# mic-rud/Learned-Compression-of-Point-Cloud-Geometry-and-Attributes

Hardware: AMD Instinct MI355X
Metric: encode+decode Mpoints/sec (higher is better)
Workload: dtype f32

## Files before the change

### include/pcc_hip.h

```cpp
#ifndef PCC_HIP_H
#define PCC_HIP_H

#include <stdint.h>

#ifdef __cplusplus
extern "C" {
#endif

#define PCC_OK 0
#define PCC_ERR_ARG (-1)
#define PCC_ERR_HIP (-2)
#define PCC_ERR_UNSUPPORTED (-3)
#define PCC_ERR_DATA (-4)

#define PCC_ACT_NONE 0
#define PCC_ACT_RELU 1
#define PCC_ACT_LEAKY_RELU 2

int pcc_version(void);
const char* pcc_last_error(void);
int pcc_device_count(void);
int pcc_device_name(int dev, char* out, int out_len);

int64_t pcc_hash_capacity(int64_t n);

#define PCC_COORD_LIMIT 130000
#define PCC_BATCH_LIMIT 1022
#define PCC_COUNT_ERR_RANGE (-2)

int pcc_hash_build(const int32_t* coords, int64_t n, uint64_t* keys, int32_t* vals, int64_t cap,
                   int32_t tensor_stride, int32_t* dup_count, void* stream);

int pcc_hash_lookup(const uint64_t* keys, const int32_t* vals, int64_t cap, int32_t tensor_stride,
                    const int32_t* query, int64_t nq, int32_t* out_idx, void* stream);

int64_t pcc_scan_scratch_elems(int64_t m);

int pcc_stride_map(const int32_t* coords, int64_t n, int32_t ts, uint64_t* keys, int32_t* vals,
                   int64_t cap, int32_t* scratch, int32_t* out_coords, int64_t* out_count,
                   void* stream);

int pcc_children(const int32_t* coords, int64_t n, int32_t ts, int32_t ksize, uint64_t* keys,
                 int32_t* vals, int64_t cap, int32_t* scratch, int32_t* out_coords,
                 int64_t* out_count, void* stream);

int pcc_augment_rotate(const int32_t* coords, int64_t n, const float* rot, int32_t nbatch, float half,
                       uint64_t* keys, int32_t* vals, int64_t cap, int32_t* scratch, int32_t* out_coords,
                       int32_t* out_src, int64_t* out_count, void* stream);

int32_t pcc_color_jitter_chunk(void);
int64_t pcc_color_jitter_scratch_bytes(int64_t n, int32_t nbatch);
int pcc_color_jitter(const float* rgb, int64_t n, const int64_t* offsets, int32_t nbatch, const float* params,
                     const int32_t* order, float* out, void* scratch, int64_t scratch_bytes, void* stream);

int pcc_voxelize(const float* xyz, const int32_t* batch, int64_t n, int32_t nbatch, const float* attr, int32_t c,
                 float origin_x, float origin_y, float origin_z, float voxel, int32_t rounding, uint64_t* keys,
                 int32_t* vals, int64_t cap, int32_t* scratch, int32_t* out_coords, int32_t* out_first,
                 int32_t* out_npts, int64_t* out_sum, int32_t* out_row, int64_t* out_count, void* stream);

int pcc_kernel_map(const int32_t* out_coords, int64_t n_out, const uint64_t* in_keys,
                   const int32_t* in_vals, int64_t in_cap, int32_t ksize, int32_t step,
                   int32_t sign, int32_t* nbr, uint32_t* row_mask, int64_t* pair_count,
                   void* stream);

int pcc_pair_count(const uint32_t* row_mask, int64_t n_out, int64_t* pair_count, void* stream);

int64_t pcc_order_scratch_bytes(int64_t n);
int pcc_order_rows_by_mask(const uint32_t* row_mask, const int32_t* coords, int64_t n,
                           int32_t block_log2, int32_t tensor_stride, int32_t* order, uint32_t* group_mask32,
                           void* scratch, int64_t scratch_bytes, void* stream);
int pcc_permute_map_rows(const int32_t* nbr, const int32_t* order, int64_t n, int32_t K, int32_t* nbr_sorted, void* stream);

int64_t pcc_small_map_max(void);
int32_t pcc_small_paths(int32_t mask);
int pcc_small_kernel_map(const int32_t* out_coords, int64_t n_out, const uint64_t* in_keys, const int32_t* in_vals, int64_t in_cap,
                         int32_t ksize, int32_t step, int32_t sign, int32_t* nbr, uint32_t* row_mask, int32_t* order,
                         uint32_t* group_mask32, void* scratch, int64_t scratch_bytes, void* stream);

int64_t pcc_conv_packed_elems(int32_t K, int32_t cin, int32_t cout);
int pcc_conv_pack_weights(const float* w, int32_t K, int32_t cin, int32_t cout, float* w_packed,
                          void* stream);
int pcc_conv_fwd(const float* fin, int64_t n_in, int32_t cin, const float* w, const float* w_packed,
                 const float* bias, const int32_t* nbr, const int32_t* order,
                 const uint32_t* group_mask32, int32_t K, float* fout, int64_t n_out, int32_t cout,
                 int32_t act, const float* film, const float* residual, void* stream);

int64_t pcc_conv_small_max(int64_t workgroups);

int pcc_conv_kernel_name(int32_t mode, int64_t n_in, int32_t cin, int32_t cout, int64_t n_out, int32_t K, int32_t has_nbr,
                         char* buf, int32_t len);

int64_t pcc_conv_packed_elems_bf16(int32_t K, int32_t cin, int32_t cout);
int pcc_conv_pack_weights_bf16(const float* w, int32_t K, int32_t cin, int32_t cout, uint16_t* w_packed, void* stream);
int pcc_conv_fwd_bf16(const uint16_t* fin, int64_t n_in, int32_t cin, const uint16_t* w_packed, const float* bias,
                      const int32_t* nbr, const int32_t* order, const uint32_t* group_mask32, int32_t K, float* fout,
                      int64_t n_out, int32_t cout, int32_t act, const float* film, const float* residual, void* stream);

int pcc_epilogue_fwd(const float* c, const float* film, const float* residual, int64_t n, int32_t channels, int32_t act,
                     float* out, void* stream);
int pcc_epilogue_bwd(const float* dout, const float* c, const float* film, int64_t n, int32_t channels, int32_t act,
                     float* dc, float* dfilm, void* stream);

int64_t pcc_cast_colsum_scratch_elems(int32_t channels);
int pcc_cast_colsum(const float* x, int64_t n, int32_t channels, uint16_t* out_bf16, float* colsum, float* scratch,
                    int64_t scratch_elems, void* stream);

int64_t pcc_conv_packed_elems_x3(int32_t K, int32_t cin, int32_t cout);
int pcc_conv_pack_weights_x3(const float* w, int32_t K, int32_t cin, int32_t cout, uint16_t* w_packed, void* stream);
int pcc_conv_fwd_x3(const float* fin, int64_t n_in, int32_t cin, const uint16_t* w_packed, const float* bias,
                    const int32_t* nbr, const int32_t* order, const uint32_t* group_mask32, int32_t K, float* fout,
                    int64_t n_out, int32_t cout, int32_t act, const float* film, const float* residual, void* stream);

int pcc_im2col_thin(const float* fin, int32_t cin, const int32_t* nbr, int64_t n_out, int32_t K, float* out, int32_t k2,
                    void* stream);

int pcc_gather_sum_fwd(const float* scores, int32_t ld, const int32_t* nbr, int32_t K, int32_t cout,
                       const float* bias, float* out, int64_t n_out, int32_t act, void* stream);

int pcc_gather_rows(const float* src, int32_t c, const int32_t* idx, int64_t n, float* out,
                    int32_t accumulate, void* stream);

int pcc_scatter_rows(const float* src, int32_t c, const int32_t* idx, int64_t n, float* out,
                     void* stream);
int pcc_scatter_add_rows(const float* src, int32_t c, const int32_t* idx, int64_t n, float* out,
                         void* stream);

int pcc_compact_rows(const uint8_t* mask, int64_t n, const int32_t* coords, int32_t* out_coords,
                     const float* feats, int32_t c, float* out_feats, int32_t* new_index,
                     int32_t* scratch, int64_t* out_count, void* stream);

int64_t pcc_topk_state_elems(int32_t nbatch);
int pcc_topk_mask(const float* logits, int32_t ld, const int32_t* coords, int64_t n, int32_t nbatch,
                  const int32_t* k, uint8_t* mask, int32_t* state, void* stream);

int pcc_count_per_batch(const int32_t* coords, int64_t n, int32_t nbatch, int32_t* counts, void* stream);

int64_t pcc_sort_scratch_bytes(int64_t n);
int pcc_sort_coords(const int32_t* coords, int64_t n, int32_t* perm, void* scratch,
                    int64_t scratch_bytes, void* stream);

int pcc_kernel_map_transpose(const int32_t* nbr, int64_t n_out, int32_t K, int64_t n_in, int32_t* nbr_t,
                             uint32_t* row_mask_t, void* stream);
int64_t pcc_conv_wgrad_scratch_elems(int32_t K, int32_t cin, int32_t cout);
int pcc_conv_wgrad(const float* fin, int64_t n_in, int32_t cin, const float* dy, int64_t n_out, int32_t cout,
                   const int32_t* nbr, const int32_t* order, const uint32_t* group_mask32, int32_t K, float* dw,
                   float* scratch, int64_t scratch_elems, void* stream);
int pcc_conv_wgrad_kernel_name(int32_t bf16, int32_t K, int32_t cin, int32_t cout, int64_t n_out, char* buf, int32_t len,
                               int32_t* split, int32_t* partials);
int pcc_conv_wgrad_bf16(const uint16_t* fin, int64_t n_in, int32_t cin, const uint16_t* dy, int64_t n_out, int32_t cout,
                        const int32_t* nbr, const int32_t* order, const uint32_t* group_mask32, int32_t K, float* dw,
                        float* scratch, int64_t scratch_elems, void* stream);

int pcc_chconv(const float* x, int64_t n, int32_t c, const int32_t* coords, const uint64_t* keys, const int32_t* vals,
               int64_t cap, int32_t tensor_stride, int32_t ksize, const float* w, int32_t w_channels, int32_t flip,
               float* y, void* stream);

int64_t pcc_octree_scratch_bytes(int64_t n);
int pcc_octree_occupancy(const int32_t* coords, int64_t n, int32_t stride, const int32_t* origin,
                         int32_t depth, uint8_t* occupancy, int32_t* level_counts, void* scratch,
                         int64_t scratch_bytes, void* stream);
int pcc_octree_expand(const uint8_t* occupancy, const int64_t* level_counts, int32_t depth,
                      int32_t stride, const int32_t* origin, int32_t batch, int64_t n_points,
                      int32_t* coords_out, void* scratch, int64_t scratch_bytes, void* stream);

int pcc_nn_search(const int32_t* query, int64_t nq, const uint64_t* keys, const int32_t* vals, int64_t cap,
                  int32_t tensor_stride, const double* target_rgb, int32_t max_radius, int32_t* nn_idx, int64_t* nn_d2,
                  int32_t* tie_count, double* tie_rgb, void* stream);

int pcc_estimate_normals(const int32_t* coords, int64_t n, const uint64_t* keys, const int32_t* vals, int64_t cap,
                         int32_t tensor_stride, int32_t radius, int32_t orient_mode, const double* orient,
                         double* normals, int32_t* count, int64_t* moments, void* stream);

int64_t pcc_render_scratch_bytes(int32_t H, int32_t W);
int pcc_render_view(const int32_t* coords, const uint8_t* rgb8, int64_t n, const int32_t* right, const int32_t* up,
                    const int32_t* front, int32_t u_min, int32_t v_max, int32_t ox, int32_t oy, int32_t scale,
                    int32_t point_size, int32_t H, int32_t W, const uint8_t* background, void* scratch,
                    int64_t scratch_bytes, uint8_t* image, void* stream);
int32_t pcc_image_compare_tile(void);
int64_t pcc_image_compare_scratch_bytes(int32_t H, int32_t W);
int pcc_image_compare(const uint8_t* ref, const uint8_t* img, int32_t H, int32_t W, void* scratch,
                      int64_t scratch_bytes, double* out, void* stream);

int pcc_eb_quantize(const float* z, int64_t n, int32_t c, const float* medians, int32_t* symbols,
                    float* z_hat, void* stream);
int pcc_eb_dequantize(const int32_t* symbols, int64_t n, int32_t c, const float* medians,
                      float* z_hat, void* stream);
int pcc_eb_likelihood(const float* z_hat, int64_t n, int32_t c, const float* eb_params, float* lik,
                      void* stream);
int pcc_gc_encode_prep(const float* y, const float* params, int64_t n, int32_t c,
                       const float* scale_table, int32_t levels, int32_t* symbols,
                       int32_t* indexes, void* stream);
int pcc_gc_encode_prep_packed(const float* y, const float* params, int64_t n, int32_t c,
                              const float* scale_table, int32_t levels, const int32_t* perm,
                              int16_t* symbols, uint8_t* indexes, int32_t* overflow, void* stream);
int pcc_gc_dequantize_i16(const int16_t* symbols, const float* params, int64_t n, int32_t c,
                          float* y_hat, void* stream);
int pcc_gc_dequantize(const int32_t* symbols, const float* params, int64_t n, int32_t c, float* y_hat,
                      void* stream);
int pcc_gc_forward(const float* y, const float* params, int64_t n, int32_t c, float* y_hat, float* lik,
                   void* stream);

int64_t pcc_rans_encode_with_indexes(const int32_t* symbols, const int32_t* indexes, int64_t n,
                                     const int32_t* cdfs, int32_t cdf_stride, const int32_t* cdf_sizes,
                                     const int32_t* offsets, uint8_t* out, int64_t out_cap);
int pcc_rans_decode_with_indexes(const uint8_t* data, int64_t nbytes, const int32_t* indexes, int64_t n,
                                 const int32_t* cdfs, int32_t cdf_stride, const int32_t* cdf_sizes,
                                 const int32_t* offsets, int32_t* out_symbols);
int64_t pcc_rans_encode_with_indexes_i16u8(const int16_t* symbols, const uint8_t* indexes, int64_t n,
                                           const int32_t* cdfs, int32_t cdf_stride, const int32_t* cdf_sizes,
                                           const int32_t* offsets, uint8_t* out, int64_t out_cap);
int pcc_rans_decode_with_indexes_u8i16(const uint8_t* data, int64_t nbytes, const uint8_t* indexes, int64_t n,
                                       const int32_t* cdfs, int32_t cdf_stride, const int32_t* cdf_sizes,
                                       const int32_t* offsets, int16_t* out_symbols, int32_t* narrowed);
int pcc_pmf_to_quantized_cdf(const float* pmf, int32_t n, int32_t precision, int32_t* cdf);

int64_t pcc_rans_lanes_header(const uint8_t* data, int64_t nbytes);
int64_t pcc_rans_lanes_encode_host(const int32_t* symbols, const int32_t* indexes, int64_t n, int32_t lanes,
                                   const int32_t* cdfs, int32_t cdf_stride, const int32_t* cdf_sizes,
                                   const int32_t* offsets, uint8_t* out, int64_t out_cap);
int pcc_rans_lanes_decode_host(const uint8_t* data, int64_t nbytes, const int32_t* indexes, int64_t n,
                               const int32_t* cdfs, int32_t cdf_stride, const int32_t* cdf_sizes,
                               const int32_t* offsets, int32_t* out_symbols);
int64_t pcc_rans_lanes_tables_bytes(const int32_t* cdf_sizes, int32_t n_tables);
int pcc_rans_lanes_tables_build(const int32_t* cdfs, int32_t cdf_stride, const int32_t* cdf_sizes,
                                const int32_t* offsets, int32_t n_tables, void* out, int64_t out_bytes);
int64_t pcc_rans_lanes_encode_scratch_bytes(int64_t n, int32_t lanes, int32_t worst_case);
int64_t pcc_rans_lanes_encode_out_bytes(int64_t n, int32_t lanes, int32_t worst_case);
int pcc_rans_lanes_encode(const int32_t* symbols, const int32_t* indexes, int64_t n, int32_t lanes,
                          const void* tables, int32_t worst_case, void* scratch, int64_t scratch_bytes,
                          uint8_t* out, int64_t out_cap, int32_t* result, void* stream);
// ... 8 lines not shown
```

### learned-compression-of-point-cloud-geometry-and-attributes_amd/_build.py

```python
import os
import subprocess

_HERE = os.path.dirname(os.path.abspath(__file__))
SO_PATH = os.path.join(_HERE, "libpcc_hip.so")

NO_SCRATCH = {
    "conv": ("conv_small_kernel", "conv_mfma_buf_kernel", "conv_mfma_kernel"),
    "rans_lanes": ("rans_lanes_encode_kernel", "rans_lanes_pack_kernel", "rans_lanes_decode_kernel"),
    "chconv": ("chconv_kernel",),
    "augment": ("jitter_partial_kernel", "jitter_mean_kernel", "jitter_apply_kernel", "first_rows_clear_kernel",
                "first_rows_insert_kernel", "first_rows_flag_kernel", "first_rows_finalize_kernel"),
    "normals": ("estimate_normals_kernel",),
    "voxelize": ("first_rows_clear_kernel", "first_rows_insert_kernel", "first_rows_flag_kernel", "first_rows_finalize_kernel",
                 "voxelize_accumulate_kernel"),
}


def build(force=False):
    args = ["make", "-s", "-C", os.path.join(_HERE, "csrc"), "-j4"]
    if force:
        subprocess.check_call(args + ["clean"])
    subprocess.check_call(args)
    for stem, kernels in NO_SCRATCH.items():
        check_kernel_resources(os.path.join(_HERE, "build", stem + ".resources.txt"), kernels)
    check_small_kernel_lds_reads()
    return SO_PATH


def check_small_kernel_lds_reads(obj=None):
    import glob
    import shutil
    objdump = "/opt/rocm/lib/llvm/bin/llvm-objdump"
    obj = obj or os.path.join(_HERE, "build", "conv.o")
    if not os.path.exists(objdump) or not os.path.exists(obj):
        raise RuntimeError(f"cannot lint conv_small_kernel: {objdump} or {obj} is missing")
    tmp = os.path.join(_HERE, "build", "_lint")
    shutil.rmtree(tmp, ignore_errors=True)
    os.makedirs(tmp)
    local = os.path.join(tmp, "conv.o")
    shutil.copy(obj, local)
    subprocess.run([objdump, "--offloading", local], check=True, capture_output=True, cwd=tmp)
    cos = [f for f in glob.glob(local + ".*") if "amdgcn" in f]
    if not cos:
        raise RuntimeError("cannot lint conv_small_kernel: no device code object in build/conv.o")
    dis = subprocess.run([objdump, "-d", cos[0]], check=True, capture_output=True, text=True).stdout
    shutil.rmtree(tmp, ignore_errors=True)
    return lint_lds_reads(dis)


def lint_lds_reads(dis, kernel="conv_small_kernel"):
    import re

    def regs(operand):
        m = re.fullmatch(r"v\[(\d+):(\d+)\]", operand)
        if m:
            return set(range(int(m.group(1)), int(m.group(2)) + 1))
        m = re.fullmatch(r"v(\d+)", operand)
        return {int(m.group(1))} if m else set()

    checked, func, pending = 0, None, {}
    for line in dis.splitlines():
        m = re.match(r"^[0-9a-f]+ <(\S+)>:", line)
        if m:
            func = m.group(1) if kernel in m.group(1) else None
            pending = {}
            continue
        if func is None:
            continue
        text = line.split("//")[0].strip()
        if not text:
            continue
        parts = text.split(None, 1)
        mnem = parts[0]
        ops = [o.strip().split(" ")[0] for o in parts[1].split(",")] if len(parts) > 1 else []
        if mnem == "s_waitcnt" and "lgkmcnt(0)" in text:
            pending = {}
            continue
        touched = set()
        for o in ops:
            touched |= regs(o)
        clash = touched & set(pending)
        if mnem == "ds_read_b128":
            dest = regs(ops[0])
            clash = (touched - dest) & set(pending) | (dest & set(pending))
            if not clash:
                for r_ in dest:
                    pending[r_] = text
                checked += 1
        if clash:
            raise RuntimeError(f"{func}: `{text}` touches v{sorted(clash)} while an LDS read into them is still in flight "
                               f"(`{pending[sorted(clash)[0]]}`): the hand-placed s_waitcnt of conv_small_kernel no longer covers it")
    if not checked:
        raise RuntimeError(f"cannot lint {kernel}: no ds_read_b128 found in its disassembly")
    return checked


def check_kernel_resources(path=None, kernels=None):
    import re
    kernels = kernels or NO_SCRATCH["conv"]
    path = path or os.path.join(_HERE, "build", "conv.resources.txt")
    if not os.path.exists(path):
        raise RuntimeError(f"{path} is missing: the library was not built by csrc/Makefile")
    seen, name = {}, None
    vals = {}
    with open(path) as f:
        for line in f:
            m = re.search(r"remark:\s+Function Name: (\S+)", line)
            if m:
                name, vals = m.group(1), {}
                seen[name] = vals
                continue
            m = re.search(r"remark:\s+(VGPRs|ScratchSize \[bytes/lane\]|SGPRs Spill|VGPRs Spill): (\d+)", line)
            if m and name:
                vals[m.group(1)] = int(m.group(2))
    bad = {k: v for k, v in seen.items() if any(t in k for t in kernels)
           and (v.get("ScratchSize [bytes/lane]", 0) or v.get("SGPRs Spill", 0) or v.get("VGPRs Spill", 0))}
    checked = [k for k in seen if any(t in k for t in kernels)]
    if not checked:
        raise RuntimeError(f"{path}: no resource remarks for {kernels} (compiler flag dropped?)")
    if bad:
        raise RuntimeError(f"kernels with scratch memory or spills (must be none): {bad}")
    return {k: (seen[k].get("VGPRs"), seen[k].get("ScratchSize [bytes/lane]")) for k in checked}
```

### learned-compression-of-point-cloud-geometry-and-attributes_amd/blocks.py

```python
import os

import torch
import torch.nn as nn

from . import _threads
from . import sparse as sp
from .sparse import (ACT_NONE, ACT_RELU, ConvChain, CoordMap, MinkowskiConvolution,
                     MinkowskiGenerativeConvolutionTranspose, MinkowskiPruning, MinkowskiReLU, SparseTensor)


class _NonNegativeParametrizer(nn.Module):
    def __init__(self, minimum=0.0, reparam_offset=2 ** -18):
        super().__init__()
        pedestal = float(reparam_offset) ** 2
        self.register_buffer("pedestal", torch.tensor([pedestal]))
        self.lower_bound = _Bound((float(minimum) + pedestal) ** 0.5)


class _Bound(nn.Module):
    def __init__(self, bound):
        super().__init__()
        self.register_buffer("bound", torch.tensor([float(bound)]))


class MinkowskiGDN(nn.Module):

    def __init__(self, in_channels, inverse=False, beta_min=1e-6, gamma_init=0.1):
        super().__init__()
        self.inverse = bool(inverse)
        self.beta_reparam = _NonNegativeParametrizer(minimum=beta_min)
        self.gamma_reparam = _NonNegativeParametrizer()
        ped = float(self.beta_reparam.pedestal)
        self.beta = nn.Parameter(torch.sqrt(torch.clamp(torch.ones(in_channels) + ped, min=ped)))
        self.gamma = nn.Parameter(torch.sqrt(torch.clamp(gamma_init * torch.eye(in_channels) + ped, min=ped)))


def _conv(cin, cout, k=3, s=1, bias=True):
    return MinkowskiConvolution(in_channels=cin, out_channels=cout, kernel_size=k, stride=s, bias=bias, dimension=3)


class ScaledBlock(nn.Module):

    def __init__(self, N, encode=True, scale=True):
        super().__init__()
        self.encode, self.scale = encode, scale
        self.conv_1 = ConvChain(_conv(N, N), MinkowskiReLU(), _conv(N, N))
        self.conv_2 = ConvChain(_conv(N, N), MinkowskiReLU(), _conv(N, N), MinkowskiReLU())
        self.gdn = MinkowskiGDN(N, inverse=(not encode))

    def forward(self, x, condition):
        if condition.map is x.map:
            film = condition.F
        else:
            film = condition.features_at_coordinates(x.C)
        N = x.F.shape[1]
        if film.shape[1] == 2 and N != 1:
            film = torch.cat([film[:, :1].expand(-1, N), film[:, 1:].expand(-1, N)], dim=1).contiguous()
        h = self.conv_1(x, last_film=film if self.scale else None)
        return self.conv_2(h, last_residual=x.F)


def _start_prefetch(x_map, done_key, job, handoffs):
    if os.environ.get("PCC_PREFETCH_MAPS", "1") == "0" or torch.is_grad_enabled() or x_map._cache.get(done_key):
        return False
    dev = x_map.device
    main = torch.cuda.current_stream(dev)
    st = _threads.current()
    skey = (dev, main.cuda_stream)
    side = st.side_streams.get(skey)
    if side is None:
        side = st.side_streams[skey] = torch.cuda.Stream(device=dev)
    x_map.table()
    side.wait_stream(main)

    def run():
        try:
            with torch.cuda.stream(side):
                job(side)
        except BaseException as e:
            for h in handoffs:
                h.fail(e)
            raise

    if x_map.n >= PREFETCH_THREAD_MIN_ROWS:
        x_map._cache[("prefetch_job",)] = st.job_thread("pcc-map-prefetch", dev).submit(run)
    else:
        run()
    x_map._cache[done_key] = True
    return True


PREFETCH_THREAD_MIN_ROWS = 8192


def prefetch_up_maps(x_map):
    first = _threads.Handoff()

    def job(side):
        cand = x_map.up(3)
        x_map.mfma_kernel_map(cand, 3, True)
        first.set(side.record_event())
        cand.mfma_kernel_map(cand, 3)
        cand.kernel_map(cand, 3)
        x_map._cache[("prefetch_event",)] = side.record_event()

    if _start_prefetch(x_map, ("okmap_prefetched",), job, [first]):
        x_map._cache[("prefetch_first",)] = first


def prefetch_analysis_maps(x_map, levels=5, hyper_ups=2):
    syncs = [_threads.Handoff() for _ in range(levels + 1)]

    def job(side):
        m, sets = x_map, [x_map]
        for lv in range(levels):
            d = m.down()
            m.mfma_kernel_map(d, 3)
            d.mfma_kernel_map(d, 3)
            sets.append(d)
            m = d
            syncs[lv].set(side.record_event())
        y_map = sets[3] if len(sets) > 3 else None
        u = m
        for _ in range(hyper_ups if y_map is not None and levels >= 5 else 0):
            c = u.up(2)
            u.mfma_kernel_map(c, 2, True)
            c.mfma_kernel_map(c, 3)
            u = c
        if y_map is not None and u is not m:
            u.mfma_kernel_map(y_map, 3)
        syncs[levels].set(side.record_event())

    if _start_prefetch(x_map, ("analysis_prefetched",), job, syncs):
        x_map._cache[("analysis_syncs",)] = syncs


def join_analysis_level(x_map, level):
    syncs = x_map._cache.get(("analysis_syncs",))
    if not syncs:
        return
    last = level == -1 or level >= len(syncs)
    try:
        ev = (syncs[-1] if last else syncs[level - 1]).wait()
    except BaseException:
        x_map._cache.pop(("analysis_syncs",), None)
        x_map._cache.pop(("prefetch_job",), None)
        raise
    torch.cuda.current_stream(x_map.device).wait_event(ev)
    if last:
        x_map._cache.pop(("analysis_syncs",), None)
        _join_prefetch(x_map)


def _join_prefetch_first(x_map):
    first = x_map._cache.pop(("prefetch_first",), None)
    if first is None:
        return
    try:
        ev = first.wait()
    except BaseException:
        x_map._cache.pop(("prefetch_job",), None)
        raise
    torch.cuda.current_stream(x_map.device).wait_event(ev)


def _join_prefetch(x_map):
    x_map._cache.pop(("prefetch_first",), None)
    done = x_map._cache.pop(("prefetch_job",), None)
    if done is not None:
        done.wait()
    ev = x_map._cache.pop(("prefetch_event",), None)
    if ev is not None:
        torch.cuda.current_stream(x_map.device).wait_event(ev)


class GenerativeUpBlock(nn.Module):

    def __init__(self, N_in, N_out, predict=False, dense=True, condition_ablation=None):
        super().__init__()
        self.dense = dense
        self.condition_ablation = condition_ablation
        self.conv = MinkowskiGenerativeConvolutionTranspose(in_channels=N_in, out_channels=N_out, kernel_size=3,
                                                            stride=2, bias=True, dimension=3)
        self.conv_2 = ConvChain(_conv(N_out, N_out), MinkowskiReLU(), _conv(N_out, N_out))
        self.prune = MinkowskiPruning()
        self.predict = predict
        if predict:
            self.occ_predict = ConvChain(_conv(N_out, N_out), MinkowskiReLU(), _conv(N_out, N_out))

    def forward(self, x, coords=None, k=None, full_predictions=False):
        if not self.predict:
            return self._follow(x, coords)
        in_map = x.map
        _join_prefetch_first(in_map)
        x = self.conv(x)
        _join_prefetch(in_map)
        if self.dense and self.condition_ablation is None:
            x = self.conv_2(x)
        pred = self.occ_predict(x, last_out_channels=None if full_predictions else 1)
        nb = x.map._nbatch if x.map._nbatch is not None else x.map.nbatch
        mask = sp.topk_mask(pred.F, pred.C, k, nb)
        kept = min(max(int(k[0]), 0), x.map.n) if nb == 1 and len(k) == 1 and not torch.is_grad_enabled() else None
        coords_kept, feats_kept, _, _ = sp.compact_rows(mask, x.C, x.F, expected=kept)
        up_map = CoordMap(coords_kept, x.map.stride, nbatch=x.map._nbatch)
        x = SparseTensor(feats_kept, coordinate_map=up_map)
        if not self.dense and self.condition_ablation is None:
            x = self.conv_2(x)
        return x, pred, up_map

    def _follow(self, Q, up_map):
        if not isinstance(up_map, CoordMap):
            up_map = CoordMap(sp._as_int_coords(up_map), Q.map.stride // 2, nbatch=Q.map._nbatch)
        return self.conv(Q, out_map=up_map)


class ConditionEncoder(nn.Module):

    def __init__(self, C_in, N_scales, N_features, condition_ablation=None):
        super().__init__()
        self.num_stages = len(N_scales)
        self.condition_ablation = condition_ablation
        self.pre_conv = ConvChain(_conv(C_in, N_features[0]), MinkowskiReLU())
        self.conv_layers = nn.ModuleList()
        self.predict_layers = nn.ModuleList()
        self.down_layers = nn.ModuleList()
        for i in range(self.num_stages):
            down = _conv(N_features[i], N_features[i + 1], 3, 2)
            self.down_layers.append(down)
            self._register_layers(down, f"down_layers_{i}")
            conv = ConvChain(_conv(N_features[i + 1], N_features[i + 1]), MinkowskiReLU(),
                             _conv(N_features[i + 1], N_features[i + 1]))
            self.conv_layers.append(conv)
            self._register_layers(conv, f"conv_layers_{i}")
            pred = ConvChain(_conv(N_features[i + 1], N_scales[i]), MinkowskiReLU(),
                             _conv(N_scales[i], N_scales[i], 1), MinkowskiReLU(),
                             _conv(N_scales[i], N_scales[i] * 2))
            self.predict_layers.append(pred)
            self._register_layers(pred, f"predict_layers_{i}")

    def _register_layers(self, layer, name):
        for pid, param in layer.named_parameters():
            self.register_parameter(f"{name}_{pid}".replace(".", "_"), param)

    def begin(self, Q):
        if self.condition_ablation not in (None, "condition_ablation"):
            raise ValueError(f"condition_ablation={self.condition_ablation!r}: the reference defines None and "
                             "'condition_ablation' only (blocks.py:244-247)")
        return self.pre_conv(Q)

    def stage(self, i, Q):
        Q = self.down_layers[i](Q)
        return Q, (self.predict_layers[i](Q) if self.condition_ablation is None else Q)

    def forward(self, Q):
        Q = self.begin(Q)
        beta_gammas = []
        for i in range(self.num_stages):
            Q, bg = self.stage(i, Q)
            beta_gammas.append(bg)
        return Q, beta_gammas
```

### learned-compression-of-point-cloud-geometry-and-attributes_amd/sparse.py

```python
import ctypes
import functools
import math
import weakref

import os

import torch
import torch.nn as nn

from . import _lib, _threads
from ._lib import PCC, check, ptr

ACT_NONE, ACT_RELU, ACT_LRELU = PCC.ACT_NONE, PCC.ACT_RELU, PCC.ACT_LEAKY_RELU


def _require_cuda(t):
    if not t.is_cuda:
        raise RuntimeError("libpcc_hip operators need tensors on an MI355X device (got a CPU tensor); "
                           "there is no CPU fallback")


COORD_PROFILER = None


def _cp_begin():
    if COORD_PROFILER is None:
        return None
    ev = torch.cuda.Event(enable_timing=True)
    ev.record()
    return ev


def _cp_end(ev0, name, rows, alg_bytes):
    if ev0 is None or COORD_PROFILER is None:
        return
    ev1 = torch.cuda.Event(enable_timing=True)
    ev1.record()
    main = torch.cuda.current_stream() == torch.cuda.default_stream()
    COORD_PROFILER.append((name, int(rows), alg_bytes, ev0, ev1, main))


def _as_int_coords(coords):
    if coords.dtype.is_floating_point:
        coords = torch.floor(coords)
    return coords.to(torch.int32).contiguous()


def _host_count():
    st = _threads.current()
    if st.count is None:
        buf = torch.zeros(1, dtype=torch.int64, pin_memory=True)
        st.count = (buf, buf.numpy())
    st.count[1][0] = COUNT_ARMED
    return st.count


_SMALL_MAP_MAX = None


def _small_map_max():
    global _SMALL_MAP_MAX
    if _SMALL_MAP_MAX is None:
        _SMALL_MAP_MAX = int(_lib.lib().pcc_small_map_max())
    return _SMALL_MAP_MAX


def set_small_map_max(rows):
    global _SMALL_MAP_MAX
    was = _small_map_max()
    _SMALL_MAP_MAX = min(int(rows), int(_lib.lib().pcc_small_map_max())) if rows else 0
    return was


def set_small_paths(mask):
    return int(_lib.lib().pcc_small_paths(int(mask)))


class CoordinateRangeError(ValueError):
    """a coordinate outside the voxel key's range (|c| <= PCC_COORD_LIMIT, 0 <= batch index <= PCC_BATCH_LIMIT: include/pcc_hip.h)"""


COUNT_ARMED, COUNT_ERR_RANGE = -1, PCC.COUNT_ERR_RANGE


def _read_count(word, device):
    import time
    deadline = time.perf_counter() + 2e-3
    while word[0] == COUNT_ARMED:
        if time.perf_counter() > deadline:
            torch.cuda.current_stream(device).synchronize()
            break
        time.sleep(0)
    n = int(word[0])
    if n == COUNT_ERR_RANGE:
        raise CoordinateRangeError(f"libpcc_hip: a voxel coordinate is outside the supported range (|c| <= {PCC.COORD_LIMIT}, batch "
                                   f"index <= {PCC.BATCH_LIMIT}): the 18-bit fields of the voxel key would alias — translate the cloud "
                                   "towards the origin or re-voxelise it")
    if n < 0:
        raise RuntimeError("libpcc_hip: the row count was never written (kernel failure?)")
    return n


def _set_buffers(m, dev):
    L = _lib.lib()
    cap = L.pcc_hash_capacity(m)
    return (torch.empty(cap, dtype=torch.int64, device=dev), torch.empty(cap, dtype=torch.int32, device=dev), cap,
            torch.empty(L.pcc_scan_scratch_elems(m), dtype=torch.int32, device=dev))


class PairCount:

    def __init__(self, row_mask):
        self._mask, self._val = row_mask, None

    def item(self):
        if self._val is None:
            out = torch.empty(1, dtype=torch.int64, device=self._mask.device)
            check(_lib.lib().pcc_pair_count(ptr(self._mask), self._mask.shape[0], ptr(out), _lib.stream()))
            self._val = int(out.item())
        return self._val

    __int__ = item

    def __float__(self):
        return float(self.item())


def _same_map(kept, out_map, self_map):
    if kept is None:
        return out_map is self_map
    return kept() is out_map


def _order_buffers(n, dev):
    return (torch.empty(n, dtype=torch.int32, device=dev), torch.empty((n + 31) // 32, dtype=torch.int32, device=dev),
            torch.empty(_lib.lib().pcc_order_scratch_bytes(n), dtype=torch.uint8, device=dev))


def _execution_order(row_mask, coords, n, stride):
    order, gmask, scratch = _order_buffers(n, coords.device)
    check(_lib.lib().pcc_order_rows_by_mask(ptr(row_mask), ptr(coords), n, ORDER_BLOCK_LOG2, stride, ptr(order), ptr(gmask),
                                            ptr(scratch), scratch.shape[0], _lib.stream()))
    return order, gmask


class CoordMap:

    def __init__(self, coords, stride=1, table=None, nbatch=None):
        _require_cuda(coords)
        assert coords.dtype == torch.int32 and coords.dim() == 2 and coords.shape[1] == 4
        self.coords = coords.contiguous()
        self.stride = int(stride)
        self._table = table
        self._nbatch = nbatch
        self._cache = {}
        self._dup_word = None

    @property
    def n(self):
        return self.coords.shape[0]

    @property
    def device(self):
        return self.coords.device

    @property
    def nbatch(self):
        if self._nbatch is None:
            self._nbatch = int(self.coords[:, 0].max().item()) + 1 if self.n else 1
        return self._nbatch

    def table(self):
        if self._table is None:
            L = _lib.lib()
            cap = L.pcc_hash_capacity(self.n)
            keys = torch.empty(cap, dtype=torch.int64, device=self.device)
            vals = torch.empty(cap, dtype=torch.int32, device=self.device)
            ev = _cp_begin()
            check(L.pcc_hash_build(ptr(self.coords), self.n, ptr(keys), ptr(vals), cap, self.stride, ptr(self._dup_word), _lib.stream()))
            _cp_end(ev, "hash_build", self.n, 28 * self.n + 12 * cap)
            self._table = (keys, vals, cap)
        return self._table

    def count_duplicates(self):
        assert self._table is None
        self._dup_word = torch.empty(1, dtype=torch.int32, device=self.device)

    def duplicates(self):
        return 0 if self._dup_word is None or self._table is None else int(self._dup_word.item())

    def lookup(self, query):
        keys, vals, cap = self.table()
        q = _as_int_coords(query)
        out = torch.empty(q.shape[0], dtype=torch.int32, device=self.device)
        ev = _cp_begin()
        check(_lib.lib().pcc_hash_lookup(ptr(keys), ptr(vals), cap, self.stride, ptr(q), q.shape[0], ptr(out), _lib.stream()))
        _cp_end(ev, "hash_lookup", q.shape[0], 32 * q.shape[0])
        return out

    def _unique(self, fn_name, m, *args):
        dev = self.device
        keys, vals, cap, scratch = _set_buffers(m, dev)
        out = torch.empty((max(m, 1), 4), dtype=torch.int32, device=dev)
        count, word = _host_count()
        ev = _cp_begin()
        check(getattr(_lib.lib(), fn_name)(ptr(self.coords), self.n, *args, ptr(keys), ptr(vals), cap, ptr(scratch),
                                           ptr(out), ptr(count), _lib.stream()))
        n_out = _read_count(word, dev)
        _cp_end(ev, "unique_" + fn_name[4:], m, 12 * cap + 16 * self.n + 12 * m + 28 * n_out)
        return out[:n_out], (keys, vals, cap)

    def down(self):
        if "down" not in self._cache:
            coords, table = self._unique("pcc_stride_map", self.n, self.stride)
            self._cache["down"] = CoordMap(coords, self.stride * 2, table, self._nbatch)
        return self._cache["down"]

    def up(self, ksize):
        key = ("up", ksize)
        if key not in self._cache:
            coords, table = self._unique("pcc_children", self.n * ksize ** 3, self.stride, ksize)
            self._cache[key] = CoordMap(coords, self.stride // 2, table, self._nbatch)
        return self._cache[key]

    def _cached_for(self, out_map, key):
        hit = self._cache.get(key)
        return hit[1:] if hit is not None and _same_map(hit[0], out_map, self) else None

    def _keep_for(self, out_map, key, *vals):
        self._cache[key] = (None if out_map is self else weakref.ref(out_map),) + vals
        return vals

    def kernel_map(self, out_map, ksize, transposed=False):
        key = ("kmap", id(out_map), ksize, transposed)
        hit = self._cached_for(out_map, key)
        if hit is not None:
            return hit
        keys, vals, cap = self.table()
        K = ksize ** 3
        n_out = out_map.n
        nbr = torch.empty((n_out, K), dtype=torch.int32, device=self.device)
        row_mask = torch.empty(n_out, dtype=torch.int32, device=self.device)
        step = self.stride // 2 if transposed else self.stride
        ev = _cp_begin()
        check(_lib.lib().pcc_kernel_map(ptr(out_map.coords), n_out, ptr(keys), ptr(vals), cap, ksize, step,
                                        -1 if transposed else 1, ptr(nbr), ptr(row_mask), None, _lib.stream()))
        pairs = PairCount(row_mask)
        probes = K * n_out if not transposed else max(n_out, K * n_out // 8)
        _cp_end(ev, "kernel_map", n_out, lambda: 20 * n_out + 8 * probes + 4 * int(pairs) + 4 * K * n_out)
        return self._keep_for(out_map, key, nbr, row_mask, pairs)

    def ordered_kernel_map(self, out_map, ksize, transposed=False):
        key = ("okmap", id(out_map), ksize, transposed, ORDER_BLOCK_LOG2)
        hit = self._cached_for(out_map, key)
        if hit is not None:
            return hit
        if (0 < out_map.n <= _small_map_max() and ksize in (2, 3) and ORDER_BLOCK_LOG2 < 0
                and ("kmap", id(out_map), ksize, transposed) not in self._cache):
            return self._small_ordered_kernel_map(out_map, ksize, transposed, key)
        nbr, row_mask, pairs = self.kernel_map(out_map, ksize, transposed)
        n_out = nbr.shape[0]
        ev = _cp_begin()
        order, gmask = _execution_order(row_mask, out_map.coords, n_out, out_map.stride)
        _cp_end(ev, "execution_order", n_out, 100 * n_out)
        return self._keep_for(out_map, key, nbr, order, gmask, pairs)

    def _small_ordered_kernel_map(self, out_map, ksize, transposed, key):
        L = _lib.lib()
        keys, vals, cap = self.table()
        n_out, K, dev = out_map.n, ksize ** 3, self.device
        nbr = torch.empty((n_out, K), dtype=torch.int32, device=dev)
        row_mask = torch.empty(n_out, dtype=torch.int32, device=dev)
        order, gmask, scratch = _order_buffers(n_out, dev)
        step = self.stride // 2 if transposed else self.stride
        ev = _cp_begin()
        check(L.pcc_small_kernel_map(ptr(out_map.coords), n_out, ptr(keys), ptr(vals), cap, ksize, step, -1 if transposed else 1,
                                     ptr(nbr), ptr(row_mask), ptr(order), ptr(gmask), ptr(scratch), scratch.shape[0], _lib.stream()))
        pairs = PairCount(row_mask)
        _cp_end(ev, "small_map+order", n_out, (120 + 12 * K) * n_out)
        self._keep_for(out_map, ("kmap", id(out_map), ksize, transposed), nbr, row_mask, pairs)
        return self._keep_for(out_map, key, nbr, order, gmask, pairs)

    def position_ordered_table(self, out_map, ksize, transposed=False):
        key = ("okmap_sorted", id(out_map), ksize, transposed, ORDER_BLOCK_LOG2)
        hit = self._cached_for(out_map, key)
        if hit is not None:
            return hit
        nbr, order, gmask, pairs = self.ordered_kernel_map(out_map, ksize, transposed)
        nbr_sorted = torch.empty_like(nbr)
        check(_lib.lib().pcc_permute_map_rows(ptr(nbr), ptr(order), nbr.shape[0], nbr.shape[1], ptr(nbr_sorted), _lib.stream()))
        return self._keep_for(out_map, key, nbr_sorted, order, gmask, pairs)

    def transposed_ordered_map(self, out_map, ksize, transposed=False):
        key = ("tmap", id(out_map), ksize, transposed, ORDER_BLOCK_LOG2)
        hit = self._cached_for(out_map, key)
        if hit is not None:
            return hit
        nbr, _, _ = self.kernel_map(out_map, ksize, transposed)
        n_out, K = nbr.shape
        nbr_t = torch.empty((self.n, K), dtype=torch.int32, device=self.device)
        mask_t = torch.empty(self.n, dtype=torch.int32, device=self.device)
        check(_lib.lib().pcc_kernel_map_transpose(ptr(nbr), n_out, K, self.n, ptr(nbr_t), ptr(mask_t), _lib.stream()))
        return self._keep_for(out_map, key, nbr_t, *_execution_order(mask_t, self.coords, self.n, self.stride))

    def conv_map(self, out_map, ksize, transposed, cin, adjoint=False):
        if ksize == 1:
            return None, None, None, None
        if adjoint:
            nbr, order, gmask = self.transposed_ordered_map(out_map, ksize, transposed)
            return (nbr, order, gmask, None) if cin % 32 == 0 else (nbr, None, None, None)
        if cin % 32 == 0:
            return self.ordered_kernel_map(out_map, ksize, transposed)
        nbr, _, pairs = self.kernel_map(out_map, ksize, transposed)
        return nbr, None, None, pairs

    def mfma_kernel_map(self, out_map, ksize, transposed=False):
        return self.ordered_kernel_map(out_map, ksize, transposed)

    def count_per_batch(self):
        if self._nbatch == 1:
            return [self.n]
        nb = self.nbatch
        counts = torch.empty(nb, dtype=torch.int32, device=self.device)
        check(_lib.lib().pcc_count_per_batch(ptr(self.coords), self.n, nb, ptr(counts), _lib.stream()))
        return [int(v) for v in counts.tolist() if v > 0]

    def sort_permutation(self):
        L = _lib.lib()
        nbytes = L.pcc_sort_scratch_bytes(self.n)
        scratch = torch.empty(nbytes, dtype=torch.uint8, device=self.device)
        perm = torch.empty(self.n, dtype=torch.int32, device=self.device)
        ev = _cp_begin()
        check(L.pcc_sort_coords(ptr(self.coords), self.n, ptr(perm), ptr(scratch), nbytes, _lib.stream()))
        _cp_end(ev, "canonical_sort", self.n, (24 + 8 * 32) * self.n)
        return perm


class SparseTensor:

    def __init__(self, features=None, coordinates=None, tensor_stride=1, coordinate_manager=None,
                 device=None, coordinate_map=None, nbatch=None):
        if coordinate_map is None:
            if coordinates is None:
                raise ValueError("coordinates or coordinate_map required")
            if device is not None:
                coordinates = coordinates.to(device)
            if isinstance(tensor_stride, (list, tuple)):
                tensor_stride = tensor_stride[0]
            coordinate_map = CoordMap(_as_int_coords(coordinates), tensor_stride, nbatch=nbatch)
        self.map = coordinate_map
        if features is None:
            features = torch.ones((self.map.n, 1), dtype=torch.float32, device=self.map.device)
        features = features.to(device=self.map.device, dtype=torch.float32)
        if features.shape[0] != self.map.n:
            raise ValueError(f"{features.shape[0]} feature rows for {self.map.n} coordinates")
        self.F = features.contiguous()

    @classmethod
    def _wrap(cls, feats, coordinate_map):
        t = object.__new__(cls)
        t.map = coordinate_map
        t.F = feats
        return t

    @property
    def C(self):
        return self.map.coords

    @property
    def tensor_stride(self):
        return [self.map.stride] * 3

    @property
    def coordinate_manager(self):
        return self.map

    @property
    def device(self):
        return self.F.device

    @property
    def shape(self):
        return self.F.shape

    def features_at_coordinates(self, query):
        idx = self.map.lookup(query)
        return gather_rows(self.F, idx)


def _tracked(*tensors):
    return torch.is_grad_enabled() and any(t is not None and t.requires_grad for t in tensors)


class _GatherRowsFn(torch.autograd.Function):

    @staticmethod
    def forward(ctx, src, idx):
        src = src.contiguous()
        n, c = idx.shape[0], src.shape[1]
        out = torch.empty((n, c), dtype=torch.float32, device=src.device)
        check(_lib.lib().pcc_gather_rows(ptr(src), c, ptr(idx), n, ptr(out), 0, _lib.stream()))
        ctx.save_for_backward(idx)
        ctx.rows = src.shape[0]
        return out

    @staticmethod
    def backward(ctx, g):
        (idx,) = ctx.saved_tensors
        g = g.contiguous()
        d = torch.zeros((ctx.rows, g.shape[1]), dtype=torch.float32, device=g.device)
        check(_lib.lib().pcc_scatter_add_rows(ptr(g), g.shape[1], ptr(idx), idx.shape[0], ptr(d), _lib.stream()))
        return d, None


def gather_rows(src, idx, out=None, accumulate=False):
    if _tracked(src, out):
        sel = _GatherRowsFn.apply(src, idx.contiguous())
        return out + sel if (accumulate and out is not None) else sel
# ... 494 lines not shown
```

### learned-compression-of-point-cloud-geometry-and-attributes_amd/transforms.py

```python
import torch
import torch.nn as nn

from . import sparse as sp
from .blocks import join_analysis_level, prefetch_analysis_maps, prefetch_up_maps, ConditionEncoder, GenerativeUpBlock, ScaledBlock, _conv
from .sparse import ConvChain, CoordMap, MinkowskiConvolution, MinkowskiReLU, SparseTensor


def _align(Q, target_map):
    if Q.map is target_map:
        return Q
    if Q.map.n != target_map.n or Q.map.stride != target_map.stride:
        return None
    idx = target_map.lookup(Q.C)
    if not bool((idx >= 0).all()):
        return None
    return SparseTensor(sp.scatter_rows(Q.F, idx, target_map.n), coordinate_map=target_map)


class AnalysisTransform(nn.Module):

    def __init__(self, config):
        super().__init__()
        C_in, N1, N2, N3 = config["C_in"], config["N1"], config["N2"], config["N3"]
        self.condition_ablation = config.get("condition_ablation")
        if config["source_condition"]:
            self.cond_conv = ConvChain(_conv(C_in, 2), MinkowskiReLU(), _conv(2, 2))
        else:
            self.cond_conv = None
        self.pre_conv = ConvChain(_conv(C_in, N1), MinkowskiReLU())
        self.down_1 = _conv(N1, N2, 3, 2)
        self.down_2 = _conv(N2, N3, 3, 2)
        self.down_3 = _conv(N3, N3, 3, 2)
        self.scale_1 = ScaledBlock(N2, encode=True, scale=True)
        self.scale_2 = ScaledBlock(N3, encode=True, scale=True)
        self.scale_3 = ScaledBlock(N3, encode=True, scale=True)
        self.post_conv = _conv(N3, N3)
        self.condition_encoder = ConditionEncoder(C_in=2, N_scales=[N2, N2, N3], N_features=[2, 2, 2, 2],
                                                  condition_ablation=self.condition_ablation)

    def count_per_batch(self, x):
        return x.map.count_per_batch()

    def forward(self, x, Q):
        k = [self.count_per_batch(x)]
        aligned = _align(Q, x.map)
        if aligned is not None:
            Q = aligned
        if self.cond_conv:
            Q_plus = self.cond_conv(x)
            if Q.map is x.map:
                Q = SparseTensor(Q.F + Q_plus.F, coordinate_map=x.map)
            else:
                Q = SparseTensor(Q.F + Q_plus.features_at_coordinates(Q.C), coordinate_map=Q.map)
        x_in_map = x.map
        prefetched = Q.map is x_in_map
        if prefetched:
            prefetch_analysis_maps(x_in_map)
        x = self.pre_conv(x)
        ce = self.condition_encoder
        Q = ce.begin(Q)
        downs, scales = (self.down_1, self.down_2, self.down_3), (self.scale_1, self.scale_2, self.scale_3)
        for i in range(3):
            if prefetched:
                join_analysis_level(x_in_map, i + 1)
            Q, beta_gamma = ce.stage(i, Q)
            x = downs[i](x)
            x = scales[i](x, beta_gamma)
            if i < 2:
                k.append(self.count_per_batch(x))
        x = self.post_conv(x)
        if prefetched:
            join_analysis_level(x_in_map, -1)

        if Q.map is x.map:
            Q8 = Q
        else:
            Q8 = SparseTensor(Q.features_at_coordinates(x.C), coordinate_map=x.map)
        k.reverse()
        return x, Q8, k


class SparseSynthesisTransform(nn.Module):

    def __init__(self, config):
        super().__init__()
        C_out, N1, N2, N3 = config["C_out"], config["N1"], config["N2"], config["N3"]
        dense = config.get("dense", True)
        if config["source_condition"]:
            self.cond_conv = ConvChain(_conv(N1, N1 // 2), MinkowskiReLU(), _conv(N1 // 2, 2))
        else:
            self.cond_conv = None
        self.pre_conv = ConvChain(_conv(N1, N1), MinkowskiReLU())
        self.up_1 = GenerativeUpBlock(N1, N1, predict=True, dense=dense)
        self.up_2 = GenerativeUpBlock(N1, N2, predict=True, dense=dense)
        self.up_3 = GenerativeUpBlock(N2, N3, predict=True, dense=dense)
        self.scale_1 = ScaledBlock(N1, encode=False, scale=True)
        self.scale_2 = ScaledBlock(N1, encode=False, scale=True)
        self.scale_3 = ScaledBlock(N2, encode=False, scale=True)
        self.post_conv = ConvChain(_conv(N3, N3), MinkowskiReLU(), _conv(N3, N3 // 2), MinkowskiReLU(),
                                   _conv(N3 // 2, C_out))
        self.q_pre_conv = ConvChain(_conv(2, 16), MinkowskiReLU(), _conv(16, 16, 1), MinkowskiReLU(), _conv(16, 2))
        self.condition_ablation = config.get("condition_ablation")
        self.q_up_1 = GenerativeUpBlock(2, 2, condition_ablation=self.condition_ablation)
        self.q_up_2 = GenerativeUpBlock(2, 2, condition_ablation=self.condition_ablation)
        self.q_up_3 = GenerativeUpBlock(2, 2, condition_ablation=self.condition_ablation)
        self.q_predict_1 = ConvChain(_conv(2, N1), MinkowskiReLU(), _conv(N1, N1), MinkowskiReLU(), _conv(N1, N1 * 2))
        self.q_predict_2 = ConvChain(_conv(2, N1), MinkowskiReLU(), _conv(N1, N1), MinkowskiReLU(), _conv(N1, N1 * 2))
        self.q_predict_3 = ConvChain(_conv(2, N2), MinkowskiReLU(), _conv(N2, N2), MinkowskiReLU(), _conv(N2, N2 * 2))
        self.down_conv = MinkowskiConvolution(in_channels=1, out_channels=1, kernel_size=3, stride=2, dimension=3)

    def forward(self, x, Q, coords=None, k=None):
        full_pred = coords is not None
        aligned = _align(Q, x.map)
        if aligned is not None:
            Q = aligned
        if self.cond_conv:
            Q_plus = self.cond_conv(x)
            if Q.map is x.map:
                Q = SparseTensor(Q.F + Q_plus.F, coordinate_map=Q.map)
            else:
                feats = sp.gather_rows(Q_plus.F, Q_plus.map.lookup(Q.C), out=Q.F.clone(), accumulate=True)
                Q = SparseTensor(feats, coordinate_map=Q.map)

        x = self.pre_conv(x)
        Q = self.q_pre_conv(Q)

        predictions = []
        ups = (self.up_1, self.up_2, self.up_3)
        q_ups = (self.q_up_1, self.q_up_2, self.q_up_3)
        q_predicts = (self.q_predict_1, self.q_predict_2, self.q_predict_3)
        scales = (self.scale_1, self.scale_2, self.scale_3)
        for i in range(3):
            prefetch_up_maps(x.map)
            beta_gamma = q_predicts[i](Q, last_out_map=x.map)
            x = scales[i](x, beta_gamma)
            x, pred, up_map = ups[i](x, k=k[i], full_predictions=full_pred)
            Q = q_ups[i](Q, up_map)
            predictions.append(pred)

        x = self.post_conv(x)

        if coords is not None:
            points_1 = coords.map.down()
            points_2 = points_1.down()
            points = [SparseTensor(coordinate_map=points_2), SparseTensor(coordinate_map=points_1), coords]
            return x, points, predictions
        return x
```

Baseline: 9.032.

## Derive pruned up-block kernel maps by restricting the candidate map on device

After top-k pruning in a generative up block, the new map's submanifold kernel map, and the follow-up transposed map, are built by a new HIP kernel. It restricts the already-cached candidate-level neighbour map through the compaction index, instead of rebuilding the hash table and running a fresh neighbour search. Hash-table construction for the pruned map becomes lazy and thread-safe, with cross-stream event waits. The last Q up-block, whose output is never used, is skipped. This adds a status word in pinned host memory for device-side guard errors, plus more cache bookkeeping that could go stale if map identity assumptions break.

```diff
diff --git a/include/pcc_hip.h b/include/pcc_hip.h
--- a/include/pcc_hip.h
+++ b/include/pcc_hip.h
@@ -76,6 +76,11 @@
 int pcc_small_kernel_map(const int32_t* out_coords, int64_t n_out, const uint64_t* in_keys, const int32_t* in_vals, int64_t in_cap,
                          int32_t ksize, int32_t step, int32_t sign, int32_t* nbr, uint32_t* row_mask, int32_t* order,
                          uint32_t* group_mask32, void* scratch, int64_t scratch_bytes, void* stream);
+
+int pcc_restrict_kernel_map(const int32_t* nbr_c, int64_t n_c, int32_t K, const int32_t* new_index_out,
+                            const int32_t* new_index_in, int64_t n_in, int64_t n_k, int32_t* nbr_k, uint32_t* row_mask_k,
+                            uint32_t* bit_counts, void* stream);
+int pcc_submap_status(void* stream, int32_t wait);
 
 int64_t pcc_conv_packed_elems(int32_t K, int32_t cin, int32_t cout);
 int pcc_conv_pack_weights(const float* w, int32_t K, int32_t cin, int32_t cout, float* w_packed,
diff --git a/learned-compression-of-point-cloud-geometry-and-attributes_amd/_build.py b/learned-compression-of-point-cloud-geometry-and-attributes_amd/_build.py
--- a/learned-compression-of-point-cloud-geometry-and-attributes_amd/_build.py
+++ b/learned-compression-of-point-cloud-geometry-and-attributes_amd/_build.py
@@ -13,6 +13,7 @@
     "normals": ("estimate_normals_kernel",),
     "voxelize": ("first_rows_clear_kernel", "first_rows_insert_kernel", "first_rows_flag_kernel", "first_rows_finalize_kernel",
                  "voxelize_accumulate_kernel"),
+    "submap": ("restrict_map_kernel",),
 }
 
 
diff --git a/learned-compression-of-point-cloud-geometry-and-attributes_amd/blocks.py b/learned-compression-of-point-cloud-geometry-and-attributes_amd/blocks.py
--- a/learned-compression-of-point-cloud-geometry-and-attributes_amd/blocks.py
+++ b/learned-compression-of-point-cloud-geometry-and-attributes_amd/blocks.py
@@ -1,4 +1,5 @@
 import os
+import weakref
 
 import torch
 import torch.nn as nn
@@ -70,7 +71,8 @@
     side = st.side_streams.get(skey)
     if side is None:
         side = st.side_streams[skey] = torch.cuda.Stream(device=dev)
-    x_map.table()
+    if not x_map._cache.get(("submap",)):
+        x_map.table()
     side.wait_stream(main)
 
     def run():
@@ -97,6 +99,7 @@
     first = _threads.Handoff()
 
     def job(side):
+        x_map.table()
         cand = x_map.up(3)
         x_map.mfma_kernel_map(cand, 3, True)
         first.set(side.record_event())
@@ -188,7 +191,7 @@
         if predict:
             self.occ_predict = ConvChain(_conv(N_out, N_out), MinkowskiReLU(), _conv(N_out, N_out))
 
-    def forward(self, x, coords=None, k=None, full_predictions=False):
+    def forward(self, x, coords=None, k=None, full_predictions=False, follow=True):
         if not self.predict:
             return self._follow(x, coords)
         in_map = x.map
@@ -201,16 +204,41 @@
         nb = x.map._nbatch if x.map._nbatch is not None else x.map.nbatch
         mask = sp.topk_mask(pred.F, pred.C, k, nb)
         kept = min(max(int(k[0]), 0), x.map.n) if nb == 1 and len(k) == 1 and not torch.is_grad_enabled() else None
-        coords_kept, feats_kept, _, _ = sp.compact_rows(mask, x.C, x.F, expected=kept)
-        up_map = CoordMap(coords_kept, x.map.stride, nbatch=x.map._nbatch)
+        cand = x.map
+        cand_maps = cand._cached_for(cand, ("kmap", id(cand), 3, False)) if sp.SUBMAP and not torch.is_grad_enabled() else None
+        coords_kept, feats_kept, new_index, _ = sp.compact_rows(mask, x.C, x.F, want_index=cand_maps is not None, expected=kept)
+        up_map = CoordMap(coords_kept, cand.stride, nbatch=cand._nbatch)
+        if cand_maps is not None and up_map.n > 0:
+            self._restrict(cand, cand_maps[0], new_index, up_map, follow)
         x = SparseTensor(feats_kept, coordinate_map=up_map)
         if not self.dense and self.condition_ablation is None:
             x = self.conv_2(x)
         return x, pred, up_map
 
+    @staticmethod
+    def _restrict(cand, nbr_c, new_index, up_map, follow):
+        up_map.keep_restricted(up_map, 3, False, nbr_c, new_index, new_index)
+        up_map._cache[("submap",)] = True
+        if follow:
+            up_map._cache[("submap_src",)] = (weakref.ref(cand), new_index)
+
+    @staticmethod
+    def _restrict_follow(in_map, up_map):
+        src = up_map._cache.pop(("submap_src",), None)
+        if src is None or not sp.SUBMAP or torch.is_grad_enabled():
+            return
+        cand, new_index = src[0](), src[1]
+        if cand is None or in_map._cached_for(up_map, ("kmap", id(up_map), 3, True)) is not None:
+            return
+        hit = in_map._cached_for(cand, ("kmap", id(cand), 3, True))
+        if hit is not None and hit[0].shape[0] == new_index.shape[0]:
+            in_map.keep_restricted(up_map, 3, True, hit[0], new_index, None)
+
     def _follow(self, Q, up_map):
         if not isinstance(up_map, CoordMap):
             up_map = CoordMap(sp._as_int_coords(up_map), Q.map.stride // 2, nbatch=Q.map._nbatch)
+        else:
+            self._restrict_follow(Q.map, up_map)
         return self.conv(Q, out_map=up_map)
 
 
diff --git a/learned-compression-of-point-cloud-geometry-and-attributes_amd/csrc/submap.hip b/learned-compression-of-point-cloud-geometry-and-attributes_amd/csrc/submap.hip
--- /dev/null
+++ b/learned-compression-of-point-cloud-geometry-and-attributes_amd/csrc/submap.hip
@@ -0,0 +1,143 @@
+#include "common.h"
+
+#include <mutex>
+
+namespace pcc {
+
+enum : int32_t { SUBMAP_OK = 0, SUBMAP_BAD_OUT_ROW = 1, SUBMAP_BAD_NEIGHBOUR = 2, SUBMAP_BAD_IN_ROW = 3 };
+
+static std::once_flag g_status_once;
+static int32_t* g_status_word = nullptr;
+
+static int32_t* status_word() {
+    std::call_once(g_status_once, [] {
+        void* p = nullptr;
+        if (hipHostMalloc(&p, 64, hipHostMallocPortable | hipHostMallocMapped) == hipSuccess && p) {
+            *reinterpret_cast<volatile int32_t*>(p) = SUBMAP_OK;
+            g_status_word = reinterpret_cast<int32_t*>(p);
+        } else {
+            (void)hipGetLastError();
+        }
+    });
+    return g_status_word;
+}
+
+static int32_t take_status() {
+    int32_t* w = status_word();
+    if (!w) return SUBMAP_OK;
+    return __atomic_load_n(w, __ATOMIC_RELAXED) ? __atomic_exchange_n(w, (int32_t)SUBMAP_OK, __ATOMIC_RELAXED) : (int32_t)SUBMAP_OK;
+}
+
+static int report_status(int32_t code) {
+    if (code == SUBMAP_OK) return PCC_OK;
+    set_error("pcc_restrict_kernel_map: a guard was violated on the device (%s); the element was written as -1",
+              code == SUBMAP_BAD_OUT_ROW ? "new_index_out names a row >= n_k: the row was not written"
+              : code == SUBMAP_BAD_NEIGHBOUR ? "nbr_c holds a row >= n_in"
+                                             : "new_index_in holds a row >= n_k");
+    return PCC_ERR_DATA;
+}
+
+template <int K>
+__global__ __launch_bounds__(256) void restrict_map_kernel(const int32_t* __restrict__ nbr_c, int64_t n_c,
+                                                           const int32_t* __restrict__ new_out,
+                                                           const int32_t* __restrict__ new_in, uint32_t n_in, uint32_t n_k,
+                                                           int32_t* __restrict__ nbr_k, uint32_t* __restrict__ row_mask_k,
+                                                           uint32_t* __restrict__ bit_counts, int32_t* __restrict__ status) {
+    __shared__ int32_t kept_row[256];
+    __shared__ unsigned short kept_src[256];
+    __shared__ unsigned rm[256];
+    __shared__ unsigned cnt[27];
+    __shared__ int wave_kept[4];
+    const int t = threadIdx.x, lane = t & 63, wave = t >> 6;
+    const int64_t row0 = (int64_t)blockIdx.x * 256;
+    const int64_t i = row0 + t;
+    int32_t r = (i < n_c) ? new_out[i] : -1;
+    if (r >= 0 && (uint32_t)r >= n_k) {
+        *status = SUBMAP_BAD_OUT_ROW;
+        r = -1;
+    }
+    const unsigned long long keep = __ballot(r >= 0);
+    if (lane == 0) wave_kept[wave] = __popcll(keep);
+    if (t < 27) cnt[t] = 0u;
+    rm[t] = 0u;
+    __syncthreads();
+    int first = 0;
+    for (int w = 0; w < wave; ++w) first += wave_kept[w];
+    const int n_kept = wave_kept[0] + wave_kept[1] + wave_kept[2] + wave_kept[3];
+    if (n_kept == 0) return;
+    if (r >= 0) {
+        const int j = first + __popcll(keep & ((1ull << lane) - 1ull));
+        kept_row[j] = r;
+        kept_src[j] = (unsigned short)t;
+    }
+    __syncthreads();
+    const int total = n_kept * K;
+    for (int e = t; e < total; e += 256) {
+        const int j = e / K, k = e - j * K;
+        const int32_t v = nbr_c[(row0 + kept_src[j]) * K + k];
+        int32_t out = -1;
+        if (v >= 0) {
+            if ((uint32_t)v < n_in) {
+                out = new_in ? new_in[v] : v;
+                if (new_in && out >= 0 && (uint32_t)out >= n_k) {
+                    *status = SUBMAP_BAD_IN_ROW;
+                    out = -1;
+                }
+            } else {
+                *status = SUBMAP_BAD_NEIGHBOUR;
+            }
+        }
+        nbr_k[(int64_t)kept_row[j] * K + k] = out;
+        if (out >= 0) atomicOr(&rm[j], 1u << k);
+    }
+    __syncthreads();
+    const unsigned m = (t < n_kept) ? rm[t] : 0u;
+    if (t < n_kept) row_mask_k[kept_row[t]] = m;
+    if (!bit_counts) return;
+    if (wave * 64 < n_kept) {
+#pragma unroll
+        for (int b = 0; b < K; ++b) {
+            const unsigned c = (unsigned)__popcll(__ballot((m >> b) & 1u));
+            if (lane == 0 && c) atomicAdd(&cnt[b], c);
+        }
+    }
+    __syncthreads();
+    if (t < K && cnt[t]) atomicAdd(&bit_counts[t], cnt[t]);
+}
+
+}
+
+using namespace pcc;
+
+extern "C" {
+
+int pcc_restrict_kernel_map(const int32_t* nbr_c, int64_t n_c, int32_t K, const int32_t* new_index_out,
+                            const int32_t* new_index_in, int64_t n_in, int64_t n_k, int32_t* nbr_k, uint32_t* row_mask_k,
+                            uint32_t* bit_counts, void* stream) {
+    PCC_REQUIRE(K == 8 || K == 27, "pcc_restrict_kernel_map: K must be 8 or 27");
+    PCC_REQUIRE(n_c >= 0 && n_c < (1ll << 31) && n_in >= 0 && n_in < (1ll << 31) && n_k >= 0 && n_k <= n_c,
+                "pcc_restrict_kernel_map: bad row counts (n_c=%lld n_in=%lld n_k=%lld)", (long long)n_c, (long long)n_in, (long long)n_k);
+    const int rc = report_status(take_status());
+    if (rc) return rc;
+    if (n_c == 0 || n_k == 0) return PCC_OK;
+    PCC_REQUIRE(nbr_c && new_index_out && nbr_k && row_mask_k, "pcc_restrict_kernel_map: null argument");
+    int32_t* status = status_word();
+    PCC_REQUIRE(status != nullptr, "pcc_restrict_kernel_map: no page-locked status word");
+    hipStream_t st = as_stream(stream);
+    const unsigned nb = blocks_for(n_c, 256);
+    if (K == 27)
+        hipLaunchKernelGGL(restrict_map_kernel<27>, dim3(nb), dim3(256), 0, st, nbr_c, n_c, new_index_out, new_index_in, (uint32_t)n_in,
+                           (uint32_t)n_k, nbr_k, row_mask_k, bit_counts, status);
+    else
+        hipLaunchKernelGGL(restrict_map_kernel<8>, dim3(nb), dim3(256), 0, st, nbr_c, n_c, new_index_out, new_index_in, (uint32_t)n_in,
+                           (uint32_t)n_k, nbr_k, row_mask_k, bit_counts, status);
+    PCC_LAUNCH_CHECK();
+    return PCC_OK;
+}
+
+int pcc_submap_status(void* stream, int32_t wait) {
+    if (wait) PCC_CHECK_HIP(hipStreamSynchronize(as_stream(stream)));
+    return report_status(take_status());
+}
+
+}
diff --git a/learned-compression-of-point-cloud-geometry-and-attributes_amd/sparse.py b/learned-compression-of-point-cloud-geometry-and-attributes_amd/sparse.py
--- a/learned-compression-of-point-cloud-geometry-and-attributes_amd/sparse.py
+++ b/learned-compression-of-point-cloud-geometry-and-attributes_amd/sparse.py
@@ -1,6 +1,7 @@
 import ctypes
 import functools
 import math
+import threading
 import weakref
 
 import os
@@ -144,6 +145,28 @@
     return order, gmask
 
 
+SUBMAP = os.environ.get("PCC_SUBMAP", "1") != "0"
+
+
+def set_submap(enabled):
+    global SUBMAP
+    was, SUBMAP = SUBMAP, bool(enabled)
+    return was
+
+
+def restrict_kernel_map(nbr_c, new_index_out, new_index_in, n_in, n_k, want_counts=False):
+    n_c, K = nbr_c.shape
+    dev = nbr_c.device
+    nbr = torch.empty((n_k, K), dtype=torch.int32, device=dev)
+    row_mask = torch.empty(n_k, dtype=torch.int32, device=dev)
+    counts = torch.zeros(27, dtype=torch.int32, device=dev) if want_counts else None
+    ev = _cp_begin()
+    check(_lib.lib().pcc_restrict_kernel_map(ptr(nbr_c), n_c, K, ptr(new_index_out), ptr(new_index_in), n_in, n_k, ptr(nbr),
+                                             ptr(row_mask), ptr(counts), _lib.stream()))
+    _cp_end(ev, "restrict_map", n_k, 4 * n_c + (8 * K + 4 + 4 * K // 3) * n_k)
+    return nbr, row_mask, counts
+
+
 class CoordMap:
 
     def __init__(self, coords, stride=1, table=None, nbatch=None):
@@ -155,6 +178,8 @@
         self._nbatch = nbatch
         self._cache = {}
         self._dup_word = None
+        self._table_lock = threading.Lock()
+        self._table_built = None
 
     @property
     def n(self):
@@ -172,15 +197,29 @@
 
     def table(self):
         if self._table is None:
-            L = _lib.lib()
-            cap = L.pcc_hash_capacity(self.n)
-            keys = torch.empty(cap, dtype=torch.int64, device=self.device)
-            vals = torch.empty(cap, dtype=torch.int32, device=self.device)
-            ev = _cp_begin()
-            check(L.pcc_hash_build(ptr(self.coords), self.n, ptr(keys), ptr(vals), cap, self.stride, ptr(self._dup_word), _lib.stream()))
-            _cp_end(ev, "hash_build", self.n, 28 * self.n + 12 * cap)
-            self._table = (keys, vals, cap)
+            with self._table_lock:
+                if self._table is None:
+                    self._build_table()
+        built = self._table_built
+        if built is not None:
+            here = _lib.stream()
+            if here not in built[0]:
+                torch.cuda.current_stream(self.device).wait_event(built[1])
+                built[0].add(here)
         return self._table
+
+    def _build_table(self):
+        L = _lib.lib()
+        cap = L.pcc_hash_capacity(self.n)
+        keys = torch.empty(cap, dtype=torch.int64, device=self.device)
+        vals = torch.empty(cap, dtype=torch.int32, device=self.device)
+        ev = _cp_begin()
+        check(L.pcc_hash_build(ptr(self.coords), self.n, ptr(keys), ptr(vals), cap, self.stride, ptr(self._dup_word), _lib.stream()))
+        _cp_end(ev, "hash_build", self.n, 28 * self.n + 12 * cap)
+        done = torch.cuda.Event()
+        done.record()
+        self._table_built = ({_lib.stream()}, done)
+        self._table = (keys, vals, cap)
 
     def count_duplicates(self):
         assert self._table is None
@@ -264,6 +303,11 @@
         order, gmask = _execution_order(row_mask, out_map.coords, n_out, out_map.stride)
         _cp_end(ev, "execution_order", n_out, 100 * n_out)
         return self._keep_for(out_map, key, nbr, order, gmask, pairs)
+
+    def keep_restricted(self, out_map, ksize, transposed, nbr_c, new_index_out, new_index_in):
+        nbr, row_mask, _ = restrict_kernel_map(nbr_c, new_index_out, new_index_in, self.n if new_index_in is None else
+                                               new_index_in.shape[0], out_map.n)
+        return self._keep_for(out_map, ("kmap", id(out_map), ksize, transposed), nbr, row_mask, PairCount(row_mask))
 
     def _small_ordered_kernel_map(self, out_map, ksize, transposed, key):
         L = _lib.lib()
diff --git a/learned-compression-of-point-cloud-geometry-and-attributes_amd/transforms.py b/learned-compression-of-point-cloud-geometry-and-attributes_amd/transforms.py
--- a/learned-compression-of-point-cloud-geometry-and-attributes_amd/transforms.py
+++ b/learned-compression-of-point-cloud-geometry-and-attributes_amd/transforms.py
@@ -134,8 +134,9 @@
             prefetch_up_maps(x.map)
             beta_gamma = q_predicts[i](Q, last_out_map=x.map)
             x = scales[i](x, beta_gamma)
-            x, pred, up_map = ups[i](x, k=k[i], full_predictions=full_pred)
-            Q = q_ups[i](Q, up_map)
+            x, pred, up_map = ups[i](x, k=k[i], full_predictions=full_pred, follow=i < 2)
+            if i < 2:
+                Q = q_ups[i](Q, up_map)
             predictions.append(pred)
 
         x = self.post_conv(x)
```

After: 9.122 (median of 6 runs). No clear change (+1.0%).
